# sunhui-3D/3D-PointCloudReconstruction

Hardware: NVIDIA B200
Metric: chamfer_fwd_bwd_point_pairs_per_s (higher is better)
Workload: dtype f32

## Files before the change

3d-pointcloudreconstruction_b200/_lib.py:

```python
import ctypes
import os

import torch

_HERE = os.path.dirname(os.path.abspath(__file__))
LIB_PATH = os.environ.get("PSD_B200_LIB") or os.path.join(_HERE, "libpsd_b200.so")

if not os.path.exists(LIB_PATH):
    raise ImportError(
        f"{LIB_PATH} is missing: build it with `python 3d-pointcloudreconstruction_b200/build.py` "
        "(nvcc, sm_100a). This package has no CPU or eager fallback."
    )

lib = ctypes.CDLL(LIB_PATH)

_vp = ctypes.c_void_p
_ci = ctypes.c_int
_cf = ctypes.c_float

_SIGNATURES = {
    "psd_chamfer_forward": [_vp, _vp, _ci, _ci, _ci, _vp, _vp, _vp, _vp, _vp],
    "psd_chamfer_forward_ex": [_vp, _vp, _ci, _ci, _ci, _ci, _vp, _vp, _vp, _vp, _vp, _cf, _vp, _ci, _ci, _vp],
    "psd_chamfer_forward_zero": [_vp, _vp, _ci, _ci, _ci, _ci, _vp, _vp, _vp, _vp, _vp, _cf, _vp, _vp, ctypes.c_longlong, _vp],
    "psd_chamfer_backward": [_vp] * 8 + [_ci, _ci, _ci, _vp],
# ... 15 lines not shown
    "psd_chamfer_mean_loss_backward_ex": [_vp, _vp, _vp, _vp, _vp, _vp, _vp, _ci, _ci, _ci, _ci, _ci, _vp],
    "psd_chamfer_loss_step_host": [_vp, _vp, _ci, _ci, _ci, _vp, _vp, _vp, _vp, _vp, _vp],
    "psd_chamfer_loss_step_host_ex": [_vp, _vp, _ci, _ci, _ci, _vp, _vp, _vp, _vp, _vp, _ci, _ci, _vp],
    "psd_chamfer_loss_step_pred_dev": [_vp, _ci, _vp, _ci, _ci, _ci, _vp, _vp, _ci, _ci, _vp],
    "psd_host_step_graphs": [_ci],
    "psd_emd_solo_mode": [_ci],
    "psd_emd_grid_mode": [_ci],
    "psd_chamfer_tc_ctas": [_ci],
    "psd_proj_min_dist": [_vp, _vp, _vp, _ci, _ci, _ci, _ci, _vp, _vp, _vp],
    "psd_icp_batch": [_vp, _vp, _ci, _ci, _ci, _vp, _ci, ctypes.c_double, _vp, _vp, _vp, _vp],
    "psd_nn_f64": [_vp, _vp, _ci, _ci, _ci, _ci, _vp, _vp, _vp],
    "psd_farthest_point_sample": [_vp, _ci, _ci, _ci, _ci, _vp, _vp],
    "psd_cont_proj": [_vp, _ci, _ci, _ci, _ci, ctypes.c_float, _vp, _vp],
    "psd_cont_proj_backward": [_vp, _vp, _ci, _ci, _ci, _ci, ctypes.c_float, _vp, _vp],
    "psd_debug_tc_prof": [_vp],
    "psd_debug_tc_filter": [_vp, _vp, _ci, _ci, _ci, _vp, _vp, _vp, _vp, _vp, _ci, _vp],
}
lib.psd_version.restype = _ci
lib.psd_last_error.restype = ctypes.c_char_p
for _n, _a in _SIGNATURES.items():
    getattr(lib, _n).argtypes = _a
    getattr(lib, _n).restype = _ci

EXPORTS = ("psd_version", "psd_last_error") + tuple(_SIGNATURES)


def last_error() -> str:
    return lib.psd_last_error().decode("utf-8", "replace")


# ... 25 lines not shown
```

3d-pointcloudreconstruction_b200/build.py:

```python
import os
import subprocess
import sys

HERE = os.path.dirname(os.path.abspath(__file__))
CSRC = os.path.join(HERE, "csrc")
OUT = os.path.join(HERE, "libpsd_b200.so")
SOURCES = ["chamfer.cu", "chamfer_nn_tc.cu", "emd.cu", "proj.cu", "icp.cu", "fps.cu", "splat.cu", "psd_capi.cu"]
NVCC_FLAGS = [
    "-gencode", "arch=compute_100a,code=sm_100a",
    "-O3", "-lineinfo", "-std=c++17",
    "-Xcompiler", "-fPIC", "-shared",
]


def needs_build() -> bool:
    if not os.path.exists(OUT):
        return True
    t = os.path.getmtime(OUT)
    deps = [os.path.join(CSRC, f) for f in os.listdir(CSRC)] + [os.path.join(HERE, "..", "include", "psd_b200.h")]
    return any(os.path.getmtime(d) > t for d in deps)


def build(force: bool = False, verbose: bool = False, out: str = OUT, defines=()) -> str:
    if out == OUT and not force and not needs_build():
# ... 36 lines not shown
```

3d-pointcloudreconstruction_b200/csrc/chamfer.cu:

```cuda
#include "chamfer_nn.cuh"
#include "psd_device.h"

#ifndef PSD_GRAD_TRIGGER_EARLY
#define PSD_GRAD_TRIGGER_EARLY 1
#endif
namespace psd {

constexpr int kWarps = 16;
constexpr int kThreads = kWarps * 32;
constexpr int kPartBytes = kWarps * kQB * 12;

__device__ unsigned long long g_fallback_queries = 0ull;

struct BlockInfo {
    int blk, d, cloud, qblock;
    float cx, cy, cz;
    float t2max;
    int bad;
    int pad[3];
};
constexpr int kPerBlockBytes = kPartBytes + (int)sizeof(BlockInfo) + 3 * kQB * 4 + kQB * 4;

template <int TM>
__global__ void __launch_bounds__(kThreads, 1) chamfer_nn_kernel(const NNParams p) {
// ... 503 lines not shown
}

}

using namespace psd;

static std::atomic<int> g_nn_variant{0};
static std::atomic<float *> g_tc_dbg{nullptr};
static std::atomic<int> g_tc_dbg_ld{0};
static std::atomic<long long *> g_tc_prof{nullptr};

bool psd_nn_tc_supported(const NNParams &p);
cudaError_t psd_launch_nn_tc(const NNParams &p, DeviceState *ds, cudaStream_t stream, float *dbg, int dbg_ld, long long *prof, int b);
void psd_set_tc_prof(long long *prof) { g_tc_prof.store(prof); }
cudaError_t psd_read_chamfer_stats_tc(unsigned long long *fallback, int reset);
void psd_set_tc_debug(float *dbg, int ld) { g_tc_dbg_ld.store(ld); g_tc_dbg.store(dbg); }

int psd_set_nn_variant(int v) {
    if (v == 0 || v == 1 || v == 3) return g_nn_variant.exchange(v);
    return g_nn_variant.load();
}

static inline void layout_strides(int layout, int bit, int npts, long long &ps, long long &cs) {
    if (layout & bit) { ps = 1; cs = npts; } else { ps = 3; cs = 1; }
}

cudaError_t psd_launch_chamfer_forward(const float *xyz1, const float *xyz2, int b, int n, int m, int layout,
                                       float *dist1, float *dist2, int *idx1, int *idx2, float *sums, float fs_thr,
                                       int *fs_count, int q_begin, int q_count, cudaStream_t stream, float *zero_buf,
                                       long long zero_floats) {
    if (zero_floats <= 0) zero_buf = nullptr;
    auto only_zero = [&]() { return zero_buf ? cudaMemsetAsync(zero_buf, 0, sizeof(float) * (size_t)zero_floats, stream) : cudaSuccess; };
    if (b <= 0 || n <= 0 || m <= 0) return only_zero();
    cudaError_t derr = cudaSuccess;
// ... 15 lines not shown
        D.qblocks = (qc + QB - 1) / QB;
        D.ntt = 1; D.ws = nullptr;
    };
    fill(p.dir[0], xyz1, n, 1, xyz2, m, 2, dist1, idx1, 0);
    fill(p.dir[1], xyz2, m, 2, xyz1, n, 1, dist2, idx2, 1);
    const long long blocks = (long long)b * (p.dir[0].qblocks + p.dir[1].qblocks);
    if (blocks == 0) return only_zero();
    if (blocks > 0x3fffffffLL) return cudaErrorInvalidConfiguration;
    p.zero_buf = zero_buf; p.zero_floats = zero_floats;
    p.pdl_trigger = 0;
    p.blocks_dir0 = b * p.dir[0].qblocks;
    p.total_blocks = (int)blocks;
    p.sums = sums; p.fs_count = fs_count; p.fs_thr = fs_thr;
    p.tile = 0; p.flush = 0;
    const int variant = g_nn_variant.load();
    if ((variant == 3 || (variant == 0 && blocks >= 2LL * num_sms)) && psd_nn_tc_supported(p)) {
        float *dbg = g_tc_dbg.exchange(nullptr);
        return psd_launch_nn_tc(p, ds, stream, dbg, g_tc_dbg_ld.load(), g_tc_prof.load(), b);
    }
    const int grid = blocks < num_sms ? (int)blocks : num_sms;
    const int per_cta = (int)((blocks + grid - 1) / grid);
    int tile = 1024;
    const int tmax = n > m ? n : m;
    while (tile < tmax && tile < 4096) tile *= 2;
    const size_t fixed = (size_t)tile * 16 + 2048;
    const size_t per_block = (size_t)kPerBlockBytes;
    int flush = (int)(((size_t)max_smem - fixed) / per_block);
    if (flush > per_cta) flush = per_cta;
    if (flush < 1) flush = 1;
    p.tile = tile; p.flush = flush;
    const size_t smem = (size_t)tile * 16 + (size_t)flush * per_block + 64;
// ... 45 lines not shown
    chamfer_grad_kernel<2><<<(unsigned int)blocks, 256, 0, stream>>>(p);
    chamfer_grad_kernel<3><<<(unsigned int)blocks, 256, 0, stream>>>(p);
    return cudaGetLastError();
}

cudaError_t psd_read_chamfer_stats(unsigned long long *fallback, int reset) {
    cudaError_t e = cudaMemcpyFromSymbol(fallback, g_fallback_queries, sizeof(unsigned long long));
    if (e != cudaSuccess) return e;
    if (reset) {
        const unsigned long long z = 0;
        e = cudaMemcpyToSymbol(g_fallback_queries, &z, sizeof(z));
        if (e != cudaSuccess) return e;
    }
    unsigned long long fg = 0;
    e = psd_read_chamfer_stats_tc(&fg, reset);
    *fallback += fg;
    return e;
}
```

3d-pointcloudreconstruction_b200/csrc/chamfer_nn_tc.cu:

```cuda
#include <cuda_fp16.h>
#include "chamfer_nn.cuh"
#include "psd_device.h"

namespace psd {
namespace tc {

#ifndef PSD_TC_SCAN_WARPS
#define PSD_TC_SCAN_WARPS 8
#endif
#ifndef PSD_TC_SETMAXNREG
#define PSD_TC_SETMAXNREG (PSD_TC_SCAN_WARPS == 16)
#endif
#ifndef PSD_TC_STAGE_FIRST
#define PSD_TC_STAGE_FIRST 0
#endif
#ifndef PSD_TC_TAIL_FAST
#define PSD_TC_TAIL_FAST 1
#endif
#ifndef PSD_TC_ALT_UNROLL
#define PSD_TC_ALT_UNROLL 2
#endif
#ifndef PSD_TC_SCAN_ALT
#define PSD_TC_SCAN_ALT 1
#endif
// ... 162 lines not shown
}
__device__ __forceinline__ float min32(const uint32_t (&r)[32]) {
    float m[4];
#pragma unroll
    for (int i = 0; i < 4; ++i) {
        m[i] = fmin3(__uint_as_float(r[8 * i]), __uint_as_float(r[8 * i + 1]), __uint_as_float(r[8 * i + 2]));
        m[i] = fmin3(m[i], __uint_as_float(r[8 * i + 3]), __uint_as_float(r[8 * i + 4]));
        m[i] = fmin3(m[i], __uint_as_float(r[8 * i + 5]), __uint_as_float(r[8 * i + 6]));
    }
    float v = fmin3(m[0], m[1], m[2]);
    v = fmin3(v, m[3], __uint_as_float(r[7]));
    v = fmin3(v, __uint_as_float(r[15]), __uint_as_float(r[23]));
    return fminf(v, __uint_as_float(r[31]));
}

struct Unit {
    int d, cloud, qblock;
    int ttile, t0, nt;
};
__device__ __forceinline__ Unit decode_unit(const NNParams &p, int blk) {
    Unit u;
    u.d = blk >= p.blocks_dir0 ? 1 : 0;
    const NNDirection &D = p.dir[u.d];
    const int bid = u.d ? blk - p.blocks_dir0 : blk;
    const int per_cloud = D.qblocks * D.ntt;
    u.cloud = bid / per_cloud;
    const int rem = bid - u.cloud * per_cloud;
    u.ttile = D.ntt == 1 ? 0 : rem / D.qblocks;
    u.qblock = rem - u.ttile * D.qblocks;
    u.t0 = u.ttile * kMaxT;
    u.nt = min(kMaxT, D.nt - u.t0);
    return u;
}
__device__ __forceinline__ void advance_unit(const NNParams &p, Unit &u, int blk_next) {
// ... 9 lines not shown
__device__ __forceinline__ int group_of(const NNParams &p, const Unit &u) { return u.d * 0x40000000 + u.cloud * p.dir[u.d].ntt + u.ttile; }
__device__ __forceinline__ const float *targets_of(const NNParams &p, const Unit &u) {
    const NNDirection &D = p.dir[u.d];
    return D.t + (long long)u.cloud * D.t_bs + (long long)u.t0 * D.t_ps;
}
__device__ __forceinline__ void store_result(const NNDirection &D, const Unit &u, int j, float dist, int idx_local) {
    if (D.ws) atomicMin(D.ws + (long long)u.cloud * D.nq + j, pack_key(dist, u.t0 + idx_local));
    else { D.dist[(long long)u.cloud * D.nq + j] = dist; D.idx[(long long)u.cloud * D.nq + j] = u.t0 + idx_local; }
}

struct Frame {
    float cx, cy, cz, cs, wmax;
    int bad, bsel;
};

struct FbQuery {
    Unit u;
    int j, nt, res;
    float x1, y1, z1;
    bool nan_possible;
    const float *bx, *by, *bz;
    long long ps;
};
__device__ __forceinline__ FbQuery fallback_query(const NNParams &p, int blk_begin, int e, const float *sraw, const int *s_rawgroup,
                                                  const float *fq) {
    FbQuery q;
    q.u = decode_unit(p, blk_begin + ((e & 0x3fffffff) >> 8));
    const NNDirection &D = p.dir[q.u.d];
    q.nt = q.u.nt;
    q.j = D.q_begin + q.u.qblock * kQB + (e & 0xff);
    q.x1 = fq[0]; q.y1 = fq[kFbCap]; q.z1 = fq[2 * kFbCap];
    q.nan_possible = ((e >> 30) & 1) || !(fabsf(q.x1) < 1e18f) || !(fabsf(q.y1) < 1e18f) || !(fabsf(q.z1) < 1e18f);
    const int grp = group_of(p, q.u);
    q.res = s_rawgroup[0] == grp ? 0 : (s_rawgroup[1] == grp ? 1 : -1);
    if (q.res >= 0) { q.bx = sraw + (q.res * 3) * kMaxT; q.by = q.bx + kMaxT; q.bz = q.by + kMaxT; q.ps = 1; }
    else { q.bx = targets_of(p, q.u); q.by = q.bx + D.t_cs; q.bz = q.by + D.t_cs; q.ps = D.t_ps; }
    return q;
}
__device__ __forceinline__ unsigned long long fallback_scan(const FbQuery &q, int part, int nsplit, int lane) {
    const float x1 = q.x1, y1 = q.y1, z1 = q.z1;
    const int nt = q.nt;
    unsigned long long key = ~0ull;
    if (q.res >= 0 && !q.nan_possible) {
        float dbest = 3.0e38f;
        int ibest = 0x7fffffff;
        for (int k0 = 4 * lane + 128 * part; k0 < nt; k0 += 128 * nsplit) {
            const float4 xa = *reinterpret_cast<const float4 *>(q.bx + k0), ya = *reinterpret_cast<const float4 *>(q.by + k0),
                         za = *reinterpret_cast<const float4 *>(q.bz + k0);
            const float d0 = sqdist_exact(xa.x - x1, ya.x - y1, za.x - z1), d1 = sqdist_exact(xa.y - x1, ya.y - y1, za.y - z1);
            const float d2 = sqdist_exact(xa.z - x1, ya.z - y1, za.z - z1), d3 = sqdist_exact(xa.w - x1, ya.w - y1, za.w - z1);
            if (d0 < dbest) { dbest = d0; ibest = k0; }
            if (k0 + 1 < nt && d1 < dbest) { dbest = d1; ibest = k0 + 1; }
            if (k0 + 2 < nt && d2 < dbest) { dbest = d2; ibest = k0 + 2; }
            if (k0 + 3 < nt && d3 < dbest) { dbest = d3; ibest = k0 + 3; }
        }
        if (ibest != 0x7fffffff) key = pack_key(dbest, ibest);
    } else {
        for (int kb = lane + 256 * part; kb < nt; kb += 256 * nsplit) {
            float dd[8], dts[8];
#pragma unroll
            for (int q8 = 0; q8 < 8; ++q8) {
                const long long k = min(kb + q8 * 32, nt - 1);
                dd[q8] = sqdist_exact(q.bx[k * q.ps] - x1, q.by[k * q.ps] - y1, q.bz[k * q.ps] - z1);
                const long long kt = k & ~(long long)(kRefTile - 1);
                dts[q8] = q.nan_possible ? sqdist_exact(q.bx[kt * q.ps] - x1, q.by[kt * q.ps] - y1, q.bz[kt * q.ps] - z1) : 0.f;
            }
#pragma unroll
            for (int q8 = 0; q8 < 8; ++q8) {
                const int k = kb + q8 * 32;
                if (k < nt && !(dd[q8] != dd[q8]) && !(dts[q8] != dts[q8])) {
                    const unsigned long long kk = pack_key(dd[q8], k);
                    key = kk < key ? kk : key;
                }
            }
        }
    }
#pragma unroll
    for (int o = 16; o > 0; o >>= 1) {
        const unsigned long long other = shfl_xor_u64(key, o);
        key = other < key ? other : key;
    }
    return key;
}
__device__ __forceinline__ void fallback_write(const NNParams &p, const FbQuery &q, unsigned long long key) {
    const NNDirection &D = p.dir[q.u.d];
    if (D.ws) {
        if (key != ~0ull) atomicMin(D.ws + (long long)q.u.cloud * D.nq + q.j, key + (unsigned long long)q.u.t0);
        return;
    }
    const float d0 = sqdist_exact(q.bx[0] - q.x1, q.by[0] - q.y1, q.bz[0] - q.z1);
    float dres;
    int ires;
    if (d0 != d0) { dres = d0; ires = 0; }
    else { dres = __uint_as_float((unsigned int)(key >> 32)); ires = (int)(key & 0xffffffffu); }
    D.dist[(long long)q.u.cloud * D.nq + q.j] = dres;
    D.idx[(long long)q.u.cloud * D.nq + q.j] = ires;
    if (p.sums) atomicAdd(p.sums + q.u.cloud * 2 + D.slot, dres);
    if (p.fs_count && dres < p.fs_thr) atomicAdd(p.fs_count + q.u.cloud * 2 + D.slot, 1);
}
__device__ __forceinline__ void run_fallbacks(const NNParams &p, int blk_begin, const int *fb_list, const float *fb_q, int nfb, int wi, int nw,
                                              int lane, const float *sraw, const int *s_rawgroup) {
    for (int fi = wi; fi < nfb; fi += nw) {
        const FbQuery q = fallback_query(p, blk_begin, fb_list[fi], sraw, s_rawgroup, fb_q + fi);
        const unsigned long long key = fallback_scan(q, 0, 1, lane);
        if (lane == 0) fallback_write(p, q, key);
    }
}

template <bool DBG>
__global__ void __launch_bounds__(kThreadsTC, 1) chamfer_nn_tc_kernel(const NNParams p, float *dbg, int dbg_ld, long long *prof) {
    extern __shared__ __align__(128) unsigned char smem[];
    float *sraw = reinterpret_cast<float *>(smem + kOffRaw);
    float *part = reinterpret_cast<float *>(smem + kOffPart);
// ... 761 lines not shown
```

3d-pointcloudreconstruction_b200/csrc/psd_capi.cu:

```cuda
#include <stdio.h>
#include <stdlib.h>
#include <string.h>

#include "../../include/psd_b200.h"
#include "psd_common.cuh"
#include "psd_device.h"

cudaError_t psd_launch_chamfer_forward(const float *xyz1, const float *xyz2, int b, int n, int m, int layout,
                                       float *dist1, float *dist2, int *idx1, int *idx2, float *sums, float fs_thr,
                                       int *fs_count, int q_begin, int q_count, cudaStream_t stream, float *zero_buf = nullptr,
                                       long long zero_floats = 0);
cudaError_t psd_launch_chamfer_backward(const float *xyz1, const float *xyz2, float *gradxyz1, float *gradxyz2,
                                        const float *graddist1, const float *graddist2, const int *idx1, const int *idx2,
                                        int b, int n, int m, int layout, int overwrite, cudaStream_t stream,
                                        const float *upstream = nullptr);
cudaError_t psd_launch_chamfer_mean_loss(const float *sums, int b, int n, int m, float *out, cudaStream_t stream);
cudaError_t psd_read_chamfer_stats(unsigned long long *fallback, int reset);
int psd_set_nn_variant(int v);
cudaError_t psd_launch_icp(const void *a, const void *b, int in_f64, int batch, int n, const double *init_pose, int max_iter,
                           double tol, double *T, double *dist, int *iters, cudaStream_t stream);
cudaError_t psd_launch_nn_f64(const void *src, const void *dst, int in_f64, int batch, int n_src, int n_dst, double *distances,
                              int *indices, cudaStream_t stream);
int psd_icp_max_points();
int psd_set_emd_solo(int enable);
int psd_set_emd_grid(int enable);
int psd_set_tc_max_ctas(int n);
cudaError_t psd_launch_cont_proj(const float *pcl, int b, int n, int grid_h, int grid_w, float sigma_sq, float *out,
                                 cudaStream_t stream);
cudaError_t psd_launch_cont_proj_backward(const float *pcl, const float *gout, int b, int n, int grid_h, int grid_w,
                                          float sigma_sq, float *gpcl, cudaStream_t stream);
cudaError_t psd_launch_fps(const float *xyz, int b, int n, int npoint, int start, long long *centroids, cudaStream_t stream);
int psd_fps_max_points();
cudaError_t psd_launch_proj_min_dist(const float *pred, const float *gt, const float *table, int b, int h, int w, int mode,
                                     float *out_min, float *out_inv, cudaStream_t stream);
void psd_set_tc_debug(float *dbg, int ld);
void psd_set_tc_prof(long long *prof);
cudaError_t psd_launch_emd_forward(const float *xyz1, const float *xyz2, int b, int n, float *dist, int *assignment,
                                   float *price, int *assignment_inv, int *bid, float *bid_increments,
                                   float *max_increments, float eps, int iters, int force_cluster, int fresh,
                                   float *loss_sums, cudaStream_t stream, int *unsupported);
cudaError_t psd_launch_emd_mean_loss(const float *sums, int b, int n, float *out, cudaStream_t stream);
cudaError_t psd_launch_emd_backward(const float *xyz1, const float *xyz2, float *gradxyz, const float *graddist,
                                    const int *idx, int b, int n, int mode, const float *upstream, cudaStream_t stream);

static thread_local char g_err[512] = "";

namespace psd {
static std::mutex g_state_mutex;
static DeviceState g_devices[kMaxDevices];
std::mutex &state_mutex() { return g_state_mutex; }
DeviceState *device_state(cudaError_t *err) {
// ... 240 lines not shown
               void *stream) {
    if (batch < 0 || n_src < 0 || n_dst < 1) { psd_set_error_msg("psd_nn_f64: batch >= 0, n_src >= 0, n_dst >= 1 required"); return -1; }
    if ((size_t)n_dst * 24 > 200 * 1024) { psd_set_error_msg("psd_nn_f64: destination cloud too large for shared memory (n_dst <= 8533)"); return -1; }
    return finish("psd_nn_f64", psd_launch_nn_f64(src, dst, in_f64, batch, n_src, n_dst, distances, indices, (cudaStream_t)stream));
}

int psd_chamfer_nn_variant(int variant) { return psd_set_nn_variant(variant); }

int psd_emd_solo_mode(int enable) { return psd_set_emd_solo(enable); }

int psd_emd_grid_mode(int enable) { return psd_set_emd_grid(enable); }

int psd_chamfer_tc_ctas(int max_ctas) { return psd_set_tc_max_ctas(max_ctas); }

int psd_debug_tc_prof(long long *prof_dev) { psd_set_tc_prof(prof_dev); return 1; }

int psd_debug_tc_filter(const float *xyz1, const float *xyz2, int b, int n, int m, float *dist1, float *dist2, int *idx1,
                        int *idx2, float *dump, int dump_ld, void *stream) {
    const int old = psd_set_nn_variant(3);
    psd_set_tc_debug(dump, dump_ld);
    cudaError_t e = psd_launch_chamfer_forward(xyz1, xyz2, b, n, m, 0, dist1, dist2, idx1, idx2, nullptr, 0.f, nullptr, 0,
                                               -1, (cudaStream_t)stream);
    psd_set_tc_debug(nullptr, 0);
    psd_set_nn_variant(old);
    return finish("psd_debug_tc_filter", e);
}

int psd_chamfer_stats(long long *out_host2, int reset) {
    unsigned long long fb = 0;
    cudaError_t e = psd_read_chamfer_stats(&fb, reset);
// ... 281 lines not shown
```

3d-pointcloudreconstruction_b200/csrc/psd_device.h:

```cpp
#pragma once
#include <cuda_runtime.h>

#include <atomic>
#include <mutex>

namespace psd {

constexpr int kMaxDevices = 64;
constexpr int kStepSlots = 8;
constexpr int kMergeSlots = 16;

struct MergeWorkspace {
    cudaStream_t stream = nullptr;
    unsigned long long *ptr = nullptr;
    size_t elems = 0;
    bool used = false;
    bool dirty = false;
    unsigned long long last_use = 0;
};

struct DeviceState {
    bool init = false;
    int device = -1;
    int num_sms = 0, max_smem = 0;
    bool attr_nn = false, attr_tc = false, attr_proj = false;
    float *fwd_ws = nullptr;
    size_t fwd_ws_bytes = 0;
    float *step_ws[kStepSlots] = {};
    size_t step_ws_bytes[kStepSlots] = {};
    MergeWorkspace merge[kMergeSlots];
    unsigned long long merge_clock = 0;
};

DeviceState *device_state(cudaError_t *err);
std::mutex &state_mutex();

}
```

include/psd_b200.h:

```cpp
#ifndef PSD_B200_H_
#define PSD_B200_H_

#ifdef __cplusplus
extern "C" {
#endif

int psd_version(void);

const char *psd_last_error(void);


int psd_chamfer_forward(const float *xyz1, const float *xyz2, int b, int n, int m, float *dist1, float *dist2,
                        int *idx1, int *idx2, void *stream);

int psd_chamfer_forward_ex(const float *xyz1, const float *xyz2, int b, int n, int m, int layout, float *dist1,
                           float *dist2, int *idx1, int *idx2, float *sums, float fs_thr, int *fs_count, int q_begin,
                           int q_count, void *stream);

int psd_chamfer_forward_zero(const float *xyz1, const float *xyz2, int b, int n, int m, int layout, float *dist1,
                             float *dist2, int *idx1, int *idx2, float *sums, float fs_thr, int *fs_count, float *zero_buf,
                             long long zero_floats, void *stream);

int psd_chamfer_backward(const float *xyz1, const float *xyz2, float *gradxyz1, float *gradxyz2,
                         const float *graddist1, const float *graddist2, const int *idx1, const int *idx2, int b, int n,
// ... 67 lines not shown
int psd_fp32_fma_peak(float ms_target, float *tflops, void *stream);

int psd_chamfer_stats(long long *out_host2, int reset);

int psd_chamfer_nn_variant(int variant);

int psd_emd_solo_mode(int enable);
int psd_emd_grid_mode(int enable);
int psd_chamfer_tc_ctas(int max_ctas);

int psd_debug_tc_filter(const float *xyz1, const float *xyz2, int b, int n, int m, float *dist1, float *dist2, int *idx1,
                        int *idx2, float *dump, int dump_ld, void *stream);

int psd_debug_tc_prof(long long *prof_dev);

#ifdef __cplusplus
}
#endif
#endif
```

Before: 7106 billion.

## Add uniform-grid spatial hashing nearest-neighbour kernel for chamfer forward

Adds a new chamfer NN kernel that bins each target cloud into a uniform 3D grid held in shared memory, sorts queries by Morton bin, and searches neighbouring cells instead of brute-forcing all targets. It becomes the default path for large launches when the grid path reports support, replacing the tensor-core brute-force kernel there. Queries with non-finite coordinates or bad bounding boxes fall back to an exact scan shared through a new header. This cuts the quadratic distance work, at the cost of grid build overhead, data-dependent load imbalance and correctness risk for non-uniform point distributions.

```diff
diff --git a/3d-pointcloudreconstruction_b200/_lib.py b/3d-pointcloudreconstruction_b200/_lib.py
--- a/3d-pointcloudreconstruction_b200/_lib.py
+++ b/3d-pointcloudreconstruction_b200/_lib.py
@@ -53,6 +53,7 @@
     "psd_cont_proj": [_vp, _ci, _ci, _ci, _ci, ctypes.c_float, _vp, _vp],
     "psd_cont_proj_backward": [_vp, _vp, _ci, _ci, _ci, _ci, ctypes.c_float, _vp, _vp],
     "psd_debug_tc_prof": [_vp],
+    "psd_debug_grid_evals": [_vp],
     "psd_debug_tc_filter": [_vp, _vp, _ci, _ci, _ci, _vp, _vp, _vp, _vp, _vp, _ci, _vp],
 }
 lib.psd_version.restype = _ci
diff --git a/3d-pointcloudreconstruction_b200/build.py b/3d-pointcloudreconstruction_b200/build.py
--- a/3d-pointcloudreconstruction_b200/build.py
+++ b/3d-pointcloudreconstruction_b200/build.py
@@ -5,7 +5,7 @@
 HERE = os.path.dirname(os.path.abspath(__file__))
 CSRC = os.path.join(HERE, "csrc")
 OUT = os.path.join(HERE, "libpsd_b200.so")
-SOURCES = ["chamfer.cu", "chamfer_nn_tc.cu", "emd.cu", "proj.cu", "icp.cu", "fps.cu", "splat.cu", "psd_capi.cu"]
+SOURCES = ["chamfer.cu", "chamfer_nn_tc.cu", "chamfer_nn_grid.cu", "emd.cu", "proj.cu", "icp.cu", "fps.cu", "splat.cu", "psd_capi.cu"]
 NVCC_FLAGS = [
     "-gencode", "arch=compute_100a,code=sm_100a",
     "-O3", "-lineinfo", "-std=c++17",
diff --git a/3d-pointcloudreconstruction_b200/csrc/chamfer.cu b/3d-pointcloudreconstruction_b200/csrc/chamfer.cu
--- a/3d-pointcloudreconstruction_b200/csrc/chamfer.cu
+++ b/3d-pointcloudreconstruction_b200/csrc/chamfer.cu
@@ -541,10 +541,13 @@
 cudaError_t psd_launch_nn_tc(const NNParams &p, DeviceState *ds, cudaStream_t stream, float *dbg, int dbg_ld, long long *prof, int b);
 void psd_set_tc_prof(long long *prof) { g_tc_prof.store(prof); }
 cudaError_t psd_read_chamfer_stats_tc(unsigned long long *fallback, int reset);
+bool psd_nn_grid_supported(const NNParams &p);
+cudaError_t psd_launch_nn_grid(const NNParams &p, DeviceState *ds, cudaStream_t stream, int b);
+cudaError_t psd_read_chamfer_stats_grid(unsigned long long *fallback, int reset);
 void psd_set_tc_debug(float *dbg, int ld) { g_tc_dbg_ld.store(ld); g_tc_dbg.store(dbg); }
 
 int psd_set_nn_variant(int v) {
-    if (v == 0 || v == 1 || v == 3) return g_nn_variant.exchange(v);
+    if (v == 0 || v == 1 || v == 3 || v == 4) return g_nn_variant.exchange(v);
     return g_nn_variant.load();
 }
 
@@ -590,7 +593,8 @@
     p.sums = sums; p.fs_count = fs_count; p.fs_thr = fs_thr;
     p.tile = 0; p.flush = 0;
     const int variant = g_nn_variant.load();
-    if ((variant == 3 || (variant == 0 && blocks >= 2LL * num_sms)) && psd_nn_tc_supported(p)) {
+    if (psd_nn_grid_supported(p) && (variant == 4 || (variant == 0 && blocks >= 2LL * num_sms))) return psd_launch_nn_grid(p, ds, stream, b);
+    if ((variant == 3 || ((variant == 0 || variant == 4) && blocks >= 2LL * num_sms)) && psd_nn_tc_supported(p)) {
         float *dbg = g_tc_dbg.exchange(nullptr);
         return psd_launch_nn_tc(p, ds, stream, dbg, g_tc_dbg_ld.load(), g_tc_prof.load(), b);
     }
@@ -666,6 +670,10 @@
     }
     unsigned long long fg = 0;
     e = psd_read_chamfer_stats_tc(&fg, reset);
+    if (e != cudaSuccess) return e;
+    *fallback += fg;
+    fg = 0;
+    e = psd_read_chamfer_stats_grid(&fg, reset);
     *fallback += fg;
     return e;
 }
diff --git a/3d-pointcloudreconstruction_b200/csrc/chamfer_nn_fallback.cuh b/3d-pointcloudreconstruction_b200/csrc/chamfer_nn_fallback.cuh
--- /dev/null
+++ b/3d-pointcloudreconstruction_b200/csrc/chamfer_nn_fallback.cuh
@@ -0,0 +1,81 @@
+#pragma once
+#include "chamfer_nn.cuh"
+
+namespace psd {
+
+struct Unit {
+    int d, cloud, qblock;
+    int ttile, t0, nt;
+};
+
+struct FbQuery {
+    Unit u;
+    int j, nt, res;
+    float x1, y1, z1;
+    bool nan_possible;
+    const float *bx, *by, *bz;
+    long long ps;
+};
+__device__ __forceinline__ unsigned long long fallback_scan(const FbQuery &q, int part, int nsplit, int lane) {
+    const float x1 = q.x1, y1 = q.y1, z1 = q.z1;
+    const int nt = q.nt;
+    unsigned long long key = ~0ull;
+    if (q.res >= 0 && !q.nan_possible) {
+        float dbest = 3.0e38f;
+        int ibest = 0x7fffffff;
+        for (int k0 = 4 * lane + 128 * part; k0 < nt; k0 += 128 * nsplit) {
+            const float4 xa = *reinterpret_cast<const float4 *>(q.bx + k0), ya = *reinterpret_cast<const float4 *>(q.by + k0),
+                         za = *reinterpret_cast<const float4 *>(q.bz + k0);
+            const float d0 = sqdist_exact(xa.x - x1, ya.x - y1, za.x - z1), d1 = sqdist_exact(xa.y - x1, ya.y - y1, za.y - z1);
+            const float d2 = sqdist_exact(xa.z - x1, ya.z - y1, za.z - z1), d3 = sqdist_exact(xa.w - x1, ya.w - y1, za.w - z1);
+            if (d0 < dbest) { dbest = d0; ibest = k0; }
+            if (k0 + 1 < nt && d1 < dbest) { dbest = d1; ibest = k0 + 1; }
+            if (k0 + 2 < nt && d2 < dbest) { dbest = d2; ibest = k0 + 2; }
+            if (k0 + 3 < nt && d3 < dbest) { dbest = d3; ibest = k0 + 3; }
+        }
+        if (ibest != 0x7fffffff) key = pack_key(dbest, ibest);
+    } else {
+        for (int kb = lane + 256 * part; kb < nt; kb += 256 * nsplit) {
+            float dd[8], dts[8];
+#pragma unroll
+            for (int q8 = 0; q8 < 8; ++q8) {
+                const long long k = min(kb + q8 * 32, nt - 1);
+                dd[q8] = sqdist_exact(q.bx[k * q.ps] - x1, q.by[k * q.ps] - y1, q.bz[k * q.ps] - z1);
+                const long long kt = k & ~(long long)(kRefTile - 1);
+                dts[q8] = q.nan_possible ? sqdist_exact(q.bx[kt * q.ps] - x1, q.by[kt * q.ps] - y1, q.bz[kt * q.ps] - z1) : 0.f;
+            }
+#pragma unroll
+            for (int q8 = 0; q8 < 8; ++q8) {
+                const int k = kb + q8 * 32;
+                if (k < nt && !(dd[q8] != dd[q8]) && !(dts[q8] != dts[q8])) {
+                    const unsigned long long kk = pack_key(dd[q8], k);
+                    key = kk < key ? kk : key;
+                }
+            }
+        }
+    }
+#pragma unroll
+    for (int o = 16; o > 0; o >>= 1) {
+        const unsigned long long other = shfl_xor_u64(key, o);
+        key = other < key ? other : key;
+    }
+    return key;
+}
+__device__ __forceinline__ void fallback_write(const NNParams &p, const FbQuery &q, unsigned long long key) {
+    const NNDirection &D = p.dir[q.u.d];
+    if (D.ws) {
+        if (key != ~0ull) atomicMin(D.ws + (long long)q.u.cloud * D.nq + q.j, key + (unsigned long long)q.u.t0);
+        return;
+    }
+    const float d0 = sqdist_exact(q.bx[0] - q.x1, q.by[0] - q.y1, q.bz[0] - q.z1);
+    float dres;
+    int ires;
+    if (d0 != d0) { dres = d0; ires = 0; }
+    else { dres = __uint_as_float((unsigned int)(key >> 32)); ires = (int)(key & 0xffffffffu); }
+    D.dist[(long long)q.u.cloud * D.nq + q.j] = dres;
+    D.idx[(long long)q.u.cloud * D.nq + q.j] = ires;
+    if (p.sums) atomicAdd(p.sums + q.u.cloud * 2 + D.slot, dres);
+    if (p.fs_count && dres < p.fs_thr) atomicAdd(p.fs_count + q.u.cloud * 2 + D.slot, 1);
+}
+
+}
diff --git a/3d-pointcloudreconstruction_b200/csrc/chamfer_nn_grid.cu b/3d-pointcloudreconstruction_b200/csrc/chamfer_nn_grid.cu
--- /dev/null
+++ b/3d-pointcloudreconstruction_b200/csrc/chamfer_nn_grid.cu
@@ -0,0 +1,395 @@
+#include "chamfer_nn.cuh"
+#include "chamfer_nn_fallback.cuh"
+#include "psd_device.h"
+
+namespace psd {
+namespace grid {
+
+constexpr int kThreads = 512;
+constexpr int kWarps = kThreads / 32;
+constexpr int kPPT = 8;
+constexpr int kMaxT = kThreads * kPPT;
+constexpr int kMaxCells = 2048;
+constexpr int kMaxG = 64;
+constexpr int kQBins = 512;
+
+__device__ unsigned long long g_fallback_queries_grid = 0ull;
+
+struct GridBox {
+    float lo[3], hi[3], h[3], inv[3], qinv[3];
+    int g[3];
+    float slack;
+    int bad;
+};
+
+__device__ __forceinline__ unsigned int ford(float f) {
+    const unsigned int u = __float_as_uint(f);
+    return (u & 0x80000000u) ? ~u : (u | 0x80000000u);
+}
+__device__ __forceinline__ float funord(unsigned int u) { return __uint_as_float((u & 0x80000000u) ? (u & 0x7fffffffu) : ~u); }
+
+__device__ __forceinline__ int axis_cell(float x, float lo, float inv, int g) {
+    return min(g - 1, max(0, __float2int_rz((x - lo) * inv)));
+}
+
+__device__ __forceinline__ void block_scan(int *a, int n, int *s_warp) {
+    const int tid = threadIdx.x, lane = tid & 31, warp = tid >> 5;
+    const int per = (n + kThreads - 1) / kThreads;
+    const int b0 = min(n, tid * per), b1 = min(n, b0 + per);
+    int loc = 0;
+    for (int i = b0; i < b1; ++i) loc += a[i];
+    int incl = loc;
+#pragma unroll
+    for (int o = 1; o < 32; o <<= 1) {
+        const int v = __shfl_up_sync(0xffffffffu, incl, o);
+        if (lane >= o) incl += v;
+    }
+    if (lane == 31) s_warp[warp] = incl;
+    __syncthreads();
+    int off = 0, tot = 0;
+#pragma unroll
+    for (int w = 0; w < kWarps; ++w) {
+        const int v = s_warp[w];
+        off += w < warp ? v : 0;
+        tot += v;
+    }
+    int run = off + incl - loc;
+    for (int i = b0; i < b1; ++i) { const int c = a[i]; a[i] = run; run += c; }
+    if (tid == 0) a[n] = tot;
+    __syncthreads();
+}
+
+__device__ __forceinline__ int morton3(int x, int y, int z) {
+    int m = 0;
+#pragma unroll
+    for (int b = 0; b < 3; ++b) m |= (((x >> b) & 1) << (3 * b)) | (((y >> b) & 1) << (3 * b + 1)) | (((z >> b) & 1) << (3 * b + 2));
+    return m;
+}
+
+template <bool EVALS>
+__global__ void __launch_bounds__(kThreads, 2) chamfer_nn_grid_kernel(const NNParams p, unsigned long long *evals) {
+    extern __shared__ __align__(16) unsigned char smem[];
+    float4 *sT = reinterpret_cast<float4 *>(smem);
+    int *cstart = reinterpret_cast<int *>(sT + p.tile);
+    int *qstart = cstart + kMaxCells + 4;
+    float4 *sQ = reinterpret_cast<float4 *>(qstart + kQBins + 4);
+    int *fbl = reinterpret_cast<int *>(sQ + kThreads);
+    int *dfl = fbl + kThreads;
+    __shared__ GridBox gb;
+    __shared__ unsigned int s_red[kWarps][7];
+    __shared__ int s_warp[kWarps];
+    __shared__ int s_nfb, s_ndf;
+
+    const int tid = threadIdx.x, lane = tid & 31, warp = tid >> 5;
+    const int G = gridDim.x;
+    const int blk_begin = (int)(((long long)blockIdx.x * p.total_blocks) / G);
+    const int blk_end = (int)(((long long)(blockIdx.x + 1) * p.total_blocks) / G);
+    pdl_wait();
+    zero_fill(p);
+
+    int res_group = -1;
+    for (int blk = blk_begin; blk < blk_end; ++blk) {
+        const int d = blk >= p.blocks_dir0 ? 1 : 0;
+        const NNDirection &D = p.dir[d];
+        const int bid = d ? blk - p.blocks_dir0 : blk;
+        const int cloud = bid / D.qblocks;
+        const int slice = bid - cloud * D.qblocks;
+        const int nt = D.nt;
+        const float *__restrict__ tb = D.t + (long long)cloud * D.t_bs;
+        const long long tps = D.t_ps, tcs = D.t_cs;
+        const int group = d * 0x40000000 + cloud;
+
+        __syncthreads();
+        for (int i = tid; i < kQBins; i += kThreads) qstart[i] = 0;
+        if (tid == 0) { s_nfb = 0; s_ndf = 0; }
+        __syncthreads();
+
+        if (group != res_group) {
+            for (int i = tid; i < kMaxCells; i += kThreads) cstart[i] = 0;
+            unsigned int mn[3] = {0xffffffffu, 0xffffffffu, 0xffffffffu}, mx[3] = {0u, 0u, 0u}, bad = 0u;
+#pragma unroll
+            for (int i = 0; i < kPPT; ++i) {
+                const int k = tid + i * kThreads;
+                if (k < nt) {
+                    const float *tp = tb + (long long)k * tps;
+                    const float c3[3] = {__ldg(tp), __ldg(tp + tcs), __ldg(tp + 2 * tcs)};
+#pragma unroll
+                    for (int a = 0; a < 3; ++a) {
+                        bad |= !(fabsf(c3[a]) < 1e18f);
+                        mn[a] = min(mn[a], ford(c3[a])); mx[a] = max(mx[a], ford(c3[a]));
+                    }
+                }
+            }
+#pragma unroll
+            for (int a = 0; a < 3; ++a) { mn[a] = __reduce_min_sync(0xffffffffu, mn[a]); mx[a] = __reduce_max_sync(0xffffffffu, mx[a]); }
+            bad = __reduce_or_sync(0xffffffffu, bad);
+            if (lane == 0) {
+#pragma unroll
+                for (int a = 0; a < 3; ++a) { s_red[warp][a] = mn[a]; s_red[warp][3 + a] = mx[a]; }
+                s_red[warp][6] = bad;
+            }
+            __syncthreads();
+            if (tid == 0) {
+                float ext[3], emax = 0.f, slack = 0.f;
+                int bd = 0;
+                for (int a = 0; a < 3; ++a) {
+                    unsigned int lo = 0xffffffffu, hi = 0u;
+                    for (int w = 0; w < kWarps; ++w) { lo = min(lo, s_red[w][a]); hi = max(hi, s_red[w][3 + a]); }
+                    gb.lo[a] = funord(lo); gb.hi[a] = funord(hi);
+                    ext[a] = gb.hi[a] - gb.lo[a];
+                    emax = fmaxf(emax, ext[a]);
+                    slack += fabsf(gb.lo[a]) + fabsf(gb.hi[a]);
+                }
+                for (int w = 0; w < kWarps; ++w) bd |= (int)s_red[w][6];
+                const int target = max(1, min(kMaxCells, nt / 2));
+                float vol = 1.f;
+                int ndim = 0;
+                bool flat[3];
+                for (int a = 0; a < 3; ++a) {
+                    flat[a] = !(ext[a] > emax * (1.0f / 1024.0f));
+                    if (!flat[a]) { vol *= ext[a] / emax; ++ndim; }
+                }
+                const float s = ndim ? powf(vol / (float)target, 1.0f / (float)ndim) : 1.f;
+                for (int a = 0; a < 3; ++a) gb.g[a] = flat[a] ? 1 : max(1, min(kMaxG, __float2int_rn((ext[a] / emax) / s)));
+                while (gb.g[0] * gb.g[1] * gb.g[2] > kMaxCells) {
+                    const int a = (gb.g[0] >= gb.g[1] && gb.g[0] >= gb.g[2]) ? 0 : (gb.g[1] >= gb.g[2] ? 1 : 2);
+                    --gb.g[a];
+                }
+                for (int a = 0; a < 3; ++a) {
+                    gb.h[a] = ext[a] / (float)gb.g[a];
+                    gb.inv[a] = (ext[a] > 0.f) ? (float)gb.g[a] / ext[a] : 0.f;
+                    gb.qinv[a] = (ext[a] > 0.f) ? 8.0f / ext[a] : 0.f;
+                }
+                gb.slack = 2e-6f * slack + 1e-36f;
+                gb.bad = bd;
+            }
+            __syncthreads();
+            const int g0 = gb.g[0], g1 = gb.g[1], g2 = gb.g[2];
+            const int nc = g0 * g1 * g2;
+            if (!gb.bad) {
+                int cr[kPPT];
+#pragma unroll
+                for (int i = 0; i < kPPT; ++i) {
+                    cr[i] = -1;
+                    const int k = tid + i * kThreads;
+                    if (k < nt) {
+                        const float *tp = tb + (long long)k * tps;
+                        const int c = (axis_cell(__ldg(tp + 2 * tcs), gb.lo[2], gb.inv[2], g2) * g1 + axis_cell(__ldg(tp + tcs), gb.lo[1], gb.inv[1], g1)) * g0 +
+                                      axis_cell(__ldg(tp), gb.lo[0], gb.inv[0], g0);
+                        cr[i] = (c << 12) | atomicAdd(cstart + c, 1);
+                    }
+                }
+                __syncthreads();
+                block_scan(cstart, nc, s_warp);
+#pragma unroll
+                for (int i = 0; i < kPPT; ++i) {
+                    if (cr[i] >= 0) {
+                        const int k = tid + i * kThreads;
+                        const float *tp = tb + (long long)k * tps;
+                        sT[cstart[cr[i] >> 12] + (cr[i] & 0xfff)] = make_float4(__ldg(tp), __ldg(tp + tcs), __ldg(tp + 2 * tcs), __int_as_float(k));
+                    }
+                }
+            }
+            res_group = group;
+        }
+
+        const int jl = tid;
+        const int j = D.q_begin + slice * kThreads + jl;
+        const bool live = j < D.q_begin + D.q_count;
+        float qx = 0.f, qy = 0.f, qz = 0.f;
+        int qbin = 0, qrank = -1;
+        if (live) {
+            const float *qp = D.q + (long long)cloud * D.q_bs + (long long)j * D.q_ps;
+            qx = __ldg(qp); qy = __ldg(qp + D.q_cs); qz = __ldg(qp + 2 * D.q_cs);
+            const bool fb = gb.bad || !(fabsf(qx) < 1e18f) || !(fabsf(qy) < 1e18f) || !(fabsf(qz) < 1e18f);
+            if (fb) {
+                fbl[atomicAdd(&s_nfb, 1)] = jl;
+            } else {
+                qbin = morton3(axis_cell(qx, gb.lo[0], gb.qinv[0], 8), axis_cell(qy, gb.lo[1], gb.qinv[1], 8),
+                               axis_cell(qz, gb.lo[2], gb.qinv[2], 8));
+                qrank = atomicAdd(qstart + qbin, 1);
+            }
+        }
+        __syncthreads();
+        block_scan(qstart, kQBins, s_warp);
+        if (qrank >= 0) sQ[qstart[qbin] + qrank] = make_float4(qx, qy, qz, __int_as_float(jl));
+        const int ng = qstart[kQBins];
+        __syncthreads();
+
+        float dres = 0.f;
+        bool settled = false;
+        if (tid < ng) {
+            const float4 Q = sQ[tid];
+            const float x1 = Q.x, y1 = Q.y, z1 = Q.z;
+            const int g0 = gb.g[0], g1 = gb.g[1], g2 = gb.g[2];
+            const int c0 = axis_cell(x1, gb.lo[0], gb.inv[0], g0), c1 = axis_cell(y1, gb.lo[1], gb.inv[1], g1),
+                      c2 = axis_cell(z1, gb.lo[2], gb.inv[2], g2);
+            const int xa = max(c0 - 1, 0), xb = min(c0 + 1, g0 - 1);
+            unsigned long long best = ~0ull;
+#pragma unroll
+            for (int dz = -1; dz <= 1; ++dz) {
+#pragma unroll
+                for (int dy = -1; dy <= 1; ++dy) {
+                    const int z = c2 + dz, y = c1 + dy;
+                    int k = 0, kend = 0;
+                    if ((unsigned)z < (unsigned)g2 && (unsigned)y < (unsigned)g1) {
+                        const int row = (z * g1 + y) * g0;
+                        k = cstart[row + xa]; kend = cstart[row + xb + 1];
+                    }
+                    if (EVALS) atomicAdd(evals, (unsigned long long)(kend - k));
+                    for (; k < kend; ++k) {
+                        const float4 t = sT[k];
+                        const float dv = sqdist_exact(t.x - x1, t.y - y1, t.z - z1);
+                        const unsigned long long key = pack_key(dv, __float_as_int(t.w));
+                        best = key < best ? key : best;
+                    }
+                }
+            }
+            const float qc[3] = {x1, y1, z1};
+            const int cc[3] = {c0, c1, c2};
+            float bx2[3];
+#pragma unroll
+            for (int a = 0; a < 3; ++a) {
+                const float gap = fmaxf(fmaxf(gb.lo[a] - qc[a], qc[a] - gb.hi[a]), 0.f);
+                bx2[a] = gap * gap;
+            }
+            float L2 = 3.0e38f;
+            bool all = true;
+#pragma unroll
+            for (int a = 0; a < 3; ++a) {
+                const int ga = a == 0 ? g0 : (a == 1 ? g1 : g2);
+                const float o2 = bx2[0] + bx2[1] + bx2[2] - bx2[a];
+                if (cc[a] - 1 > 0) {
+                    const float face = gb.lo[a] + (float)(cc[a] - 1) * gb.h[a] + gb.slack;
+                    const float gap = fmaxf(fmaxf(gb.lo[a] - qc[a], qc[a] - face), 0.f);
+                    L2 = fminf(L2, __fmaf_rn(gap, gap, o2));
+                    all = false;
+                }
+                if (cc[a] + 1 < ga - 1) {
+                    const float face = gb.lo[a] + (float)(cc[a] + 2) * gb.h[a] - gb.slack;
+                    const float gap = fmaxf(fmaxf(face - qc[a], qc[a] - gb.hi[a]), 0.f);
+                    L2 = fminf(L2, __fmaf_rn(gap, gap, o2));
+                    all = false;
+                }
+            }
+            const float dbest = __uint_as_float((unsigned int)(best >> 32));
+            settled = all || __fmaf_rn(L2, -0x1p-19f, L2) - 1e-44f > dbest;
+            if (settled) {
+                const int jq = D.q_begin + slice * kThreads + __float_as_int(Q.w);
+                dres = dbest;
+                D.dist[(long long)cloud * D.nq + jq] = dres;
+                D.idx[(long long)cloud * D.nq + jq] = (int)(best & 0xffffffffu);
+            } else {
+                dfl[atomicAdd(&s_ndf, 1)] = tid;
+            }
+            if (EVALS) {
+                atomicAdd(evals + 1, 1ull);
+                if (!settled) atomicAdd(evals + 3, 1ull);
+            }
+        }
+        if (p.sums != nullptr || p.fs_count != nullptr) {
+            float ws = settled ? dres : 0.f;
+            int wc = (settled && dres < p.fs_thr) ? 1 : 0;
+#pragma unroll
+            for (int o = 16; o > 0; o >>= 1) {
+                ws += __shfl_xor_sync(0xffffffffu, ws, o);
+                wc += __shfl_xor_sync(0xffffffffu, wc, o);
+            }
+            if (lane == 0 && warp * 32 < ng) {
+                if (p.sums) atomicAdd(p.sums + cloud * 2 + D.slot, ws);
+                if (p.fs_count && wc) atomicAdd(p.fs_count + cloud * 2 + D.slot, wc);
+            }
+        }
+        __syncthreads();
+
+        const int ndf = s_ndf;
+        for (int fi = warp; fi < ndf; fi += kWarps) {
+            const float4 Q = sQ[dfl[fi]];
+            unsigned long long best = ~0ull;
+#pragma unroll 4
+            for (int k = lane; k < nt; k += 32) {
+                const float4 t = sT[k];
+                const unsigned long long key = pack_key(sqdist_exact(t.x - Q.x, t.y - Q.y, t.z - Q.z), __float_as_int(t.w));
+                best = key < best ? key : best;
+            }
+#pragma unroll
+            for (int o = 16; o > 0; o >>= 1) {
+                const unsigned long long other = shfl_xor_u64(best, o);
+                best = other < best ? other : best;
+            }
+            if (lane == 0) {
+                const int jq = D.q_begin + slice * kThreads + __float_as_int(Q.w);
+                const float dv = __uint_as_float((unsigned int)(best >> 32));
+                D.dist[(long long)cloud * D.nq + jq] = dv;
+                D.idx[(long long)cloud * D.nq + jq] = (int)(best & 0xffffffffu);
+                if (p.sums) atomicAdd(p.sums + cloud * 2 + D.slot, dv);
+                if (p.fs_count && dv < p.fs_thr) atomicAdd(p.fs_count + cloud * 2 + D.slot, 1);
+            }
+        }
+        if (p.pdl_trigger && blk == blk_end - 1) pdl_trigger();
+
+        const int nfb = s_nfb;
+        for (int fi = warp; fi < nfb; fi += kWarps) {
+            FbQuery q;
+            q.u.d = d; q.u.cloud = cloud; q.u.qblock = slice; q.u.ttile = 0; q.u.t0 = 0; q.u.nt = nt;
+            q.j = D.q_begin + slice * kThreads + fbl[fi];
+            q.nt = nt; q.res = -1;
+            const float *qp = D.q + (long long)cloud * D.q_bs + (long long)q.j * D.q_ps;
+            q.x1 = __ldg(qp); q.y1 = __ldg(qp + D.q_cs); q.z1 = __ldg(qp + 2 * D.q_cs);
+            q.nan_possible = true;
+            q.bx = D.t + (long long)cloud * D.t_bs; q.by = q.bx + D.t_cs; q.bz = q.by + D.t_cs; q.ps = D.t_ps;
+            const unsigned long long key = fallback_scan(q, 0, 1, lane);
+            if (lane == 0) fallback_write(p, q, key);
+        }
+        if (nfb > 0 && tid == 0) atomicAdd(&g_fallback_queries_grid, (unsigned long long)nfb);
+    }
+}
+
+}
+}
+
+using namespace psd;
+
+static std::atomic<unsigned long long *> g_grid_evals{nullptr};
+void psd_set_grid_evals(unsigned long long *evals) { g_grid_evals.store(evals); }
+int psd_set_tc_max_ctas(int n);
+
+bool psd_nn_grid_supported(const NNParams &p) { return p.dir[0].nt <= grid::kMaxT && p.dir[1].nt <= grid::kMaxT; }
+
+cudaError_t psd_launch_nn_grid(const NNParams &p_in, DeviceState *ds, cudaStream_t stream, int b) {
+    const size_t smem_max = (size_t)grid::kMaxT * 16 + (size_t)(grid::kMaxCells + 4 + grid::kQBins + 4) * 4 + (size_t)grid::kThreads * 24;
+    {
+        std::lock_guard<std::mutex> lock(state_mutex());
+        if (!ds->attr_grid) {
+            cudaError_t e = cudaFuncSetAttribute(grid::chamfer_nn_grid_kernel<false>, cudaFuncAttributeMaxDynamicSharedMemorySize, (int)smem_max);
+            if (e == cudaSuccess) e = cudaFuncSetAttribute(grid::chamfer_nn_grid_kernel<true>, cudaFuncAttributeMaxDynamicSharedMemorySize, (int)smem_max);
+            if (e != cudaSuccess) return e;
+            ds->attr_grid = true;
+        }
+    }
+    NNParams p = p_in;
+    for (int d = 0; d < 2; ++d) p.dir[d].qblocks = (p.dir[d].q_count + grid::kThreads - 1) / grid::kThreads;
+    p.blocks_dir0 = b * p.dir[0].qblocks;
+    p.total_blocks = p.blocks_dir0 + b * p.dir[1].qblocks;
+    p.tile = ((p.dir[0].nt > p.dir[1].nt ? p.dir[0].nt : p.dir[1].nt) + 3) & ~3;
+    const size_t smem = (size_t)p.tile * 16 + (size_t)(grid::kMaxCells + 4 + grid::kQBins + 4) * 4 + (size_t)grid::kThreads * 24;
+    int grid_ctas = p.total_blocks;
+    const int cap = psd_set_tc_max_ctas(-1);
+    if (cap > 0 && grid_ctas > cap) grid_ctas = cap;
+    p.pdl_trigger = (cap > 0 && grid_ctas == cap) ? 0 : 1;
+    unsigned long long *evals = g_grid_evals.load();
+    if (evals)
+        return psd_launch_pdl(p.pdl_trigger != 0, grid::chamfer_nn_grid_kernel<true>, dim3(grid_ctas), dim3(grid::kThreads), smem, stream, p, evals);
+    return psd_launch_pdl(p.pdl_trigger != 0, grid::chamfer_nn_grid_kernel<false>, dim3(grid_ctas), dim3(grid::kThreads), smem, stream, p,
+                          (unsigned long long *)nullptr);
+}
+
+cudaError_t psd_read_chamfer_stats_grid(unsigned long long *fallback, int reset) {
+    cudaError_t e = cudaMemcpyFromSymbol(fallback, grid::g_fallback_queries_grid, sizeof(unsigned long long));
+    if (e != cudaSuccess) return e;
+    if (reset) {
+        const unsigned long long z = 0;
+        e = cudaMemcpyToSymbol(grid::g_fallback_queries_grid, &z, sizeof(z));
+    }
+    return e;
+}
diff --git a/3d-pointcloudreconstruction_b200/csrc/chamfer_nn_tc.cu b/3d-pointcloudreconstruction_b200/csrc/chamfer_nn_tc.cu
--- a/3d-pointcloudreconstruction_b200/csrc/chamfer_nn_tc.cu
+++ b/3d-pointcloudreconstruction_b200/csrc/chamfer_nn_tc.cu
@@ -1,5 +1,6 @@
 #include <cuda_fp16.h>
 #include "chamfer_nn.cuh"
+#include "chamfer_nn_fallback.cuh"
 #include "psd_device.h"
 
 namespace psd {
@@ -200,10 +201,6 @@
     return fminf(v, __uint_as_float(r[31]));
 }
 
-struct Unit {
-    int d, cloud, qblock;
-    int ttile, t0, nt;
-};
 __device__ __forceinline__ Unit decode_unit(const NNParams &p, int blk) {
     Unit u;
     u.d = blk >= p.blocks_dir0 ? 1 : 0;
@@ -243,14 +240,6 @@
     int bad, bsel;
 };
 
-struct FbQuery {
-    Unit u;
-    int j, nt, res;
-    float x1, y1, z1;
-    bool nan_possible;
-    const float *bx, *by, *bz;
-    long long ps;
-};
 __device__ __forceinline__ FbQuery fallback_query(const NNParams &p, int blk_begin, int e, const float *sraw, const int *s_rawgroup,
                                                   const float *fq) {
     FbQuery q;
@@ -265,67 +254,6 @@
     if (q.res >= 0) { q.bx = sraw + (q.res * 3) * kMaxT; q.by = q.bx + kMaxT; q.bz = q.by + kMaxT; q.ps = 1; }
     else { q.bx = targets_of(p, q.u); q.by = q.bx + D.t_cs; q.bz = q.by + D.t_cs; q.ps = D.t_ps; }
     return q;
-}
-__device__ __forceinline__ unsigned long long fallback_scan(const FbQuery &q, int part, int nsplit, int lane) {
-    const float x1 = q.x1, y1 = q.y1, z1 = q.z1;
-    const int nt = q.nt;
-    unsigned long long key = ~0ull;
-    if (q.res >= 0 && !q.nan_possible) {
-        float dbest = 3.0e38f;
-        int ibest = 0x7fffffff;
-        for (int k0 = 4 * lane + 128 * part; k0 < nt; k0 += 128 * nsplit) {
-            const float4 xa = *reinterpret_cast<const float4 *>(q.bx + k0), ya = *reinterpret_cast<const float4 *>(q.by + k0),
-                         za = *reinterpret_cast<const float4 *>(q.bz + k0);
-            const float d0 = sqdist_exact(xa.x - x1, ya.x - y1, za.x - z1), d1 = sqdist_exact(xa.y - x1, ya.y - y1, za.y - z1);
-            const float d2 = sqdist_exact(xa.z - x1, ya.z - y1, za.z - z1), d3 = sqdist_exact(xa.w - x1, ya.w - y1, za.w - z1);
-            if (d0 < dbest) { dbest = d0; ibest = k0; }
-            if (k0 + 1 < nt && d1 < dbest) { dbest = d1; ibest = k0 + 1; }
-            if (k0 + 2 < nt && d2 < dbest) { dbest = d2; ibest = k0 + 2; }
-            if (k0 + 3 < nt && d3 < dbest) { dbest = d3; ibest = k0 + 3; }
-        }
-        if (ibest != 0x7fffffff) key = pack_key(dbest, ibest);
-    } else {
-        for (int kb = lane + 256 * part; kb < nt; kb += 256 * nsplit) {
-            float dd[8], dts[8];
-#pragma unroll
-            for (int q8 = 0; q8 < 8; ++q8) {
-                const long long k = min(kb + q8 * 32, nt - 1);
-                dd[q8] = sqdist_exact(q.bx[k * q.ps] - x1, q.by[k * q.ps] - y1, q.bz[k * q.ps] - z1);
-                const long long kt = k & ~(long long)(kRefTile - 1);
-                dts[q8] = q.nan_possible ? sqdist_exact(q.bx[kt * q.ps] - x1, q.by[kt * q.ps] - y1, q.bz[kt * q.ps] - z1) : 0.f;
-            }
-#pragma unroll
-            for (int q8 = 0; q8 < 8; ++q8) {
-                const int k = kb + q8 * 32;
-                if (k < nt && !(dd[q8] != dd[q8]) && !(dts[q8] != dts[q8])) {
-                    const unsigned long long kk = pack_key(dd[q8], k);
-                    key = kk < key ? kk : key;
-                }
-            }
-        }
-    }
-#pragma unroll
-    for (int o = 16; o > 0; o >>= 1) {
-        const unsigned long long other = shfl_xor_u64(key, o);
-        key = other < key ? other : key;
-    }
-    return key;
-}
-__device__ __forceinline__ void fallback_write(const NNParams &p, const FbQuery &q, unsigned long long key) {
-    const NNDirection &D = p.dir[q.u.d];
-    if (D.ws) {
-        if (key != ~0ull) atomicMin(D.ws + (long long)q.u.cloud * D.nq + q.j, key + (unsigned long long)q.u.t0);
-        return;
-    }
-    const float d0 = sqdist_exact(q.bx[0] - q.x1, q.by[0] - q.y1, q.bz[0] - q.z1);
-    float dres;
-    int ires;
-    if (d0 != d0) { dres = d0; ires = 0; }
-    else { dres = __uint_as_float((unsigned int)(key >> 32)); ires = (int)(key & 0xffffffffu); }
-    D.dist[(long long)q.u.cloud * D.nq + q.j] = dres;
-    D.idx[(long long)q.u.cloud * D.nq + q.j] = ires;
-    if (p.sums) atomicAdd(p.sums + q.u.cloud * 2 + D.slot, dres);
-    if (p.fs_count && dres < p.fs_thr) atomicAdd(p.fs_count + q.u.cloud * 2 + D.slot, 1);
 }
 __device__ __forceinline__ void run_fallbacks(const NNParams &p, int blk_begin, const int *fb_list, const float *fb_q, int nfb, int wi, int nw,
                                               int lane, const float *sraw, const int *s_rawgroup) {
diff --git a/3d-pointcloudreconstruction_b200/csrc/psd_capi.cu b/3d-pointcloudreconstruction_b200/csrc/psd_capi.cu
--- a/3d-pointcloudreconstruction_b200/csrc/psd_capi.cu
+++ b/3d-pointcloudreconstruction_b200/csrc/psd_capi.cu
@@ -35,6 +35,7 @@
                                      float *out_min, float *out_inv, cudaStream_t stream);
 void psd_set_tc_debug(float *dbg, int ld);
 void psd_set_tc_prof(long long *prof);
+void psd_set_grid_evals(unsigned long long *evals);
 cudaError_t psd_launch_emd_forward(const float *xyz1, const float *xyz2, int b, int n, float *dist, int *assignment,
                                    float *price, int *assignment_inv, int *bid, float *bid_increments,
                                    float *max_increments, float eps, int iters, int force_cluster, int fresh,
@@ -305,6 +306,8 @@
 int psd_chamfer_tc_ctas(int max_ctas) { return psd_set_tc_max_ctas(max_ctas); }
 
 int psd_debug_tc_prof(long long *prof_dev) { psd_set_tc_prof(prof_dev); return 1; }
+
+int psd_debug_grid_evals(unsigned long long *evals_dev) { psd_set_grid_evals(evals_dev); return 1; }
 
 int psd_debug_tc_filter(const float *xyz1, const float *xyz2, int b, int n, int m, float *dist1, float *dist2, int *idx1,
                         int *idx2, float *dump, int dump_ld, void *stream) {
diff --git a/3d-pointcloudreconstruction_b200/csrc/psd_device.h b/3d-pointcloudreconstruction_b200/csrc/psd_device.h
--- a/3d-pointcloudreconstruction_b200/csrc/psd_device.h
+++ b/3d-pointcloudreconstruction_b200/csrc/psd_device.h
@@ -23,7 +23,7 @@
     bool init = false;
     int device = -1;
     int num_sms = 0, max_smem = 0;
-    bool attr_nn = false, attr_tc = false, attr_proj = false;
+    bool attr_nn = false, attr_tc = false, attr_grid = false, attr_proj = false;
     float *fwd_ws = nullptr;
     size_t fwd_ws_bytes = 0;
     float *step_ws[kStepSlots] = {};
diff --git a/include/psd_b200.h b/include/psd_b200.h
--- a/include/psd_b200.h
+++ b/include/psd_b200.h
@@ -105,6 +105,8 @@
 
 int psd_debug_tc_prof(long long *prof_dev);
 
+int psd_debug_grid_evals(unsigned long long *evals_dev);
+
 #ifdef __cplusplus
 }
 #endif
```

New measurement: 9121 billion, median of 6. 28.4% higher.
